# JANUS-Institute/HallThrusterPEM

Measured on AMD Instinct MI355X. Metric: coupled PEM-v0 model evals/sec, higher is better.
Workload: dtype f64

## Files before the change

### hallthrusterpem_amd/_lib.py

```python
import ctypes as C
import importlib.util
import os
import threading
from pathlib import Path

PKG = Path(__file__).resolve().parent
LIB_PATH = PKG / 'libpem_hip.so'

PEM_OK, PEM_ERR_INVALID_ARG, PEM_ERR_HIP, PEM_ERR_NO_DEVICE = 0, 1, 2, 3
NANGLE = 91
FUSED_LATENT_MAX_RANK = 8
FUSED_SYSTEM_MAX_RECORDS = 1024
FUSED_SYSTEM_MAX_RADII = 8
SYS_JION, SYS_VCC, SYS_T, SYS_UION = 0, 1, 2, 3
SWEEP_CATHODE, SWEEP_THRUSTER, SWEEP_PLUME = 0, 1, 2
DE_MAX_POP, DE_MAX_DIM = 1024, 16
DE_BEST1BIN, DE_RAND1BIN = 0, 1
CHAIN_TIME_BLOCK = 4096
MARGINALS_MAX_PAR, MARGINALS_MAX_BINS = 32, 64
HIST_ROW_TILE = 128
KDE_MAX_GRID, KDE_ROW_BLOCK = 4096, 4096

_dp = C.c_void_p
_sz = C.c_size_t
_f8 = C.c_double

SIGNATURES = {
    'pem_version': (C.c_char_p, []),
    'pem_last_error': (C.c_char_p, []),
    'pem_device_count': (C.c_int, []),
    'pem_init': (C.c_int, [C.c_int]),
    'pem_synchronize': (C.c_int, [_dp]),
    'pem_set_lanes_per_sample': (C.c_int, [C.c_int]),
    'pem_angle_grid': (C.POINTER(C.c_double), []),
    'pem_persistent_grid': (C.c_int, [_sz, C.c_int, C.c_int, C.c_int, C.POINTER(_sz), C.POINTER(_sz)]),
    'pem_coupled_occupancy': (C.c_int, [C.c_int, C.POINTER(C.c_int), C.POINTER(C.c_int)]),
    'pem_cathode_f64_dev': (C.c_int, [_sz] + [_dp] * 6 + [_f8, _dp, _dp]),
    'pem_cathode_f64': (C.c_int, [_sz] + [_dp] * 6 + [_f8, _dp]),
    'pem_plume_f64_dev': (C.c_int, [_sz, C.c_int, _dp, _f8] + [_dp] * 10 + [_dp] * 4 + [_dp]),
    'pem_plume_f64': (C.c_int, [_sz, C.c_int, _dp, _f8] + [_dp] * 10 + [_dp] * 4),
    'pem_thruster_f64_dev': (C.c_int, [_sz] + [_dp] * 4 + [_dp] * 8 + [_dp]),
    'pem_thruster_f64': (C.c_int, [_sz] + [_dp] * 4 + [_dp] * 8),
    'pem_thruster_uion_f64_dev': (C.c_int, [_sz, _dp, _f8, _f8, C.c_int, _dp, _dp, _dp]),
    'pem_thruster_filter_f64_dev': (C.c_int, [_sz, C.c_int, _dp, _dp, _f8, C.c_int, _dp, _dp, _dp, _dp]),
    'pem_coupled_f64_dev': (C.c_int, [_sz, _f8, _f8] + [_dp] * 15 + [_dp] * 7 + [_dp]),
    'pem_coupled_f64': (C.c_int, [_sz, _f8, _f8] + [_dp] * 15 + [_dp] * 7),
    'pem_coupled_tiled_f64_dev': (C.c_int, [_sz, _f8, _f8, _dp] + [_dp] * 7 + [_dp]),
    'pem_coupled_mixed_dev': (C.c_int, [_sz, _f8, _f8] + [_dp] * 15 + [_dp] * 7 + [_dp]),
    'pem_coupled_loglik_f64_dev': (C.c_int, [_sz, _f8, _f8] + [_dp] * 15 + [C.c_int, C.c_int] + [_dp] * 4 + [_dp] * 5 + [_dp]),
    'pem_coupled_system_loglik_f64_dev': (C.c_int, [_sz, _f8, _f8] + [_dp] * 15 + [C.c_int, C.c_int, _dp, _dp, C.c_int, _dp, _f8, _f8, C.c_int]
                                          + [_dp] * 5 + [_dp]),
    'pem_coupled_system_predict_f64_dev': (C.c_int, [_sz, _f8, _f8] + [_dp] * 15 + [C.c_int, C.c_int, _dp, _dp, C.c_int, _dp, _f8, _f8, C.c_int]
                                           + [_dp] * 4 + [_sz, _dp, _dp]),
    'pem_coupled_system_loglik_radii_f64_dev': (C.c_int, [_sz, _f8, C.c_int, _dp] + [_dp] * 15
                                                + [C.c_int, C.c_int, _dp, _dp, C.c_int, _dp, _f8, _f8, C.c_int] + [_dp] * 5 + [_dp]),
    'pem_coupled_system_predict_radii_f64_dev': (C.c_int, [_sz, _f8, C.c_int, _dp] + [_dp] * 15
                                                 + [C.c_int, C.c_int, _dp, _dp, C.c_int, _dp, _f8, _f8, C.c_int] + [_dp] * 4 + [_sz, _dp, _dp]),
    'pem_predictive_inputs_f64_dev': (C.c_int, [_sz, C.c_int, C.c_uint64, C.c_uint64, C.c_uint32, _dp, _dp, _dp, _dp, _dp, _sz, C.c_int,
                                                _dp, C.c_uint32, _dp, _sz, _dp]),
    'pem_predictive_noise_f64_dev': (C.c_int, [_sz, C.c_int, _dp, _sz, _dp, C.c_uint64, C.c_uint64, C.c_uint32, _dp, _sz, _dp]),
    'pem_coupled_latent_f64_dev': (C.c_int, [_sz, _f8, _f8] + [_dp] * 15 + [C.c_int, C.c_int, _dp, _dp] + [_dp] * 4 + [_dp]),
    'pem_loglik_marginal_f64_dev': (C.c_int, [_sz, C.c_int, C.c_int, _dp, _dp, _dp, _f8, _f8, _dp, _dp, _dp]),
    'pem_log_prior_f64_dev': (C.c_int, [_sz, C.c_int, _dp, _dp, _dp, _dp, _dp, _dp, _dp, _dp]),
    'pem_jion_loglik_f64_dev': (C.c_int, [_sz, C.c_int, C.c_int] + [_dp] * 6 + [_dp]),
    'pem_svd_compress_f64_dev': (C.c_int, [_sz, C.c_int, C.c_int, C.c_int, _f8, _dp, _dp, _dp, _dp]),
    'pem_svd_reconstruct_f64_dev': (C.c_int, [_sz, C.c_int, C.c_int, C.c_int, _f8, _dp, _dp, _dp, _dp]),
    'pem_coupled_mc_f64_dev': (C.c_int, [_sz, C.c_uint64, C.c_uint64, C.c_uint32, C.c_int, _dp, _dp, _dp, _f8, _f8, _dp, _sz] + [_dp] * 7 + [_dp]),
    'pem_sparse_predict_f64_dev': (C.c_int, [_sz, C.c_int, C.c_int, _dp, _dp, _dp, C.c_int, _dp, _sz, _dp, _sz, C.c_int, C.c_int, _dp]),
    'pem_sparse_grid_values_f64_dev': (C.c_int, [_sz, C.c_int, C.c_int, _dp, _dp, _dp, C.c_int, _dp, _sz, _dp, _sz, C.c_int, C.c_int, _dp]),
    'pem_sparse_predict_field_f64_dev': (C.c_int, [_sz, C.c_int, C.c_int, _dp, _dp, _dp, C.c_int, _dp, _sz, _dp, _sz, C.c_int, C.c_int,
                                                   C.c_int, C.c_int, C.c_int, C.c_int, C.c_double, _dp, _dp, _dp]),
    'pem_sparse_predict_chain_f64_dev': (C.c_int, [_sz, C.c_int, C.c_int, C.c_int, _dp, _f8, _f8, _f8, _f8, _dp, _sz, _dp, _sz,
                                                   C.c_int, C.c_int, C.c_int, C.c_int, C.c_double, _dp, _dp, _dp]),
    'pem_chain_system_loglik_f64_dev': (C.c_int, [_sz, C.c_int, C.c_int, C.c_int, _dp, _f8, _f8, _f8, _f8, _dp, _sz,
                                                  C.c_int, C.c_int, C.c_int, C.c_int, C.c_double, _dp, C.c_int, C.c_int, _dp, _dp,
                                                  _dp, _f8, _f8, _dp, _dp, _sz, _dp, _sz, _dp]),
    'pem_sparse_predict_chain_fields_f64_dev': (C.c_int, [_sz, C.c_int, C.c_int, C.c_int, _dp, _f8, _f8, _f8, _f8, _dp, _sz, _dp, _sz,
                                                          C.c_int, C.c_int, C.c_int, C.c_int, C.c_double, _dp, _dp,
                                                          C.c_int, C.c_int, C.c_int, C.c_int, C.c_double, _dp, _dp, _dp]),
    'pem_chain_fields_loglik_f64_dev': (C.c_int, [_sz, C.c_int, C.c_int, C.c_int, _dp, _f8, _f8, _f8, _f8, _dp, _sz,
                                                  C.c_int, C.c_int, C.c_int, C.c_int, C.c_double, _dp, C.c_int, C.c_int, _dp, _dp,
                                                  _dp, _f8, _f8, _dp, _dp, _sz, _dp, _sz,
                                                  C.c_int, C.c_int, C.c_int, C.c_int, C.c_double, _dp, C.c_int, _dp, _dp, _dp]),
    'pem_key_minmax_f64_dev': (C.c_int, [_sz, C.c_int, _dp, _sz, _dp, _dp, _dp, _dp]),
    'pem_range_hist_f64_dev': (C.c_int, [_sz, C.c_int, _dp, _sz, C.c_int, _dp, _dp, C.c_int, _dp, _dp]),
    'pem_range_narrow_dev': (C.c_int, [C.c_int, C.c_int, _dp, _dp, _dp, _dp, _dp]),
    'pem_qsel_bins': (C.c_int, [C.c_int, C.c_int, C.POINTER(C.c_int), C.POINTER(C.c_int)]),
    'pem_qsel_minmax_f64_dev': (C.c_int, [_sz, C.c_int, _dp, _sz, _dp, _dp, _dp, _dp]),
    'pem_qsel_hist1_f64_dev': (C.c_int, [_sz, C.c_int, _dp, _sz, _dp, _dp, C.c_int, _dp, _dp]),
# ... 71 lines not shown
        if _lib is not None:
            return _lib
        path = Path(os.environ.get('PEM_HIP_LIB', LIB_PATH))
        if 'PEM_HIP_LIB' not in os.environ:
            from . import build as _build
            if _build.needs_build():
                if _build.have_hipcc():
                    _build.build()
                elif not path.exists():
                    raise RuntimeError('libpem_hip.so is missing and hipcc is not available to build it')
                else:
                    import warnings
                    warnings.warn('libpem_hip.so is older than its sources and hipcc is not available: loading the stale library')
        _hip_runtime = _share_torch_hip_runtime()
        lib = C.CDLL(str(path))
        for name, (res, args) in SIGNATURES.items():
            fn = getattr(lib, name)
            fn.restype = res
            fn.argtypes = args
        _lib = lib
    return _lib


def check(rc: int):
    if rc != PEM_OK:
        raise PemHipError(rc, load().pem_last_error().decode(errors='replace'))


def device_count() -> int:
    return int(load().pem_device_count())


def set_device(index: int):
    check(load().pem_init(int(index)))
    try:
        import torch
        torch.cuda.set_device(int(index))
    except ImportError:
        pass


def persistent_grid(n: int, cus: int, wg_per_cu: int, memory_bound: bool = True):
    wg, spr = _sz(0), _sz(0)
    check(load().pem_persistent_grid(int(n), int(cus), int(wg_per_cu), 1 if memory_bound else 0, C.byref(wg), C.byref(spr)))
    return int(wg.value), int(spr.value)


def coupled_occupancy(profile_mode: int = 1):
    cus, per = C.c_int(0), C.c_int(0)
    check(load().pem_coupled_occupancy(int(profile_mode), C.byref(cus), C.byref(per)))
    return int(cus.value), int(per.value)


def require_device():
    if device_count() < 1:
        raise PemHipError(PEM_ERR_NO_DEVICE, 'no HIP device visible; hallthrusterpem_amd has no CPU path')
```

### hallthrusterpem_amd/csrc/pem_kernels.hip

```cpp
#include <cmath>
#include <cstdlib>
#include <atomic>
#include <mutex>
#include <type_traits>

#include "pem_math.h"
#include "pem_philox.h"
#include "pem_plume.h"

namespace {

using namespace pem;
using namespace pem_model;

struct CoupledIO {
    const double *V_a, *T_e, *V_vac, *Pstar, *P_T, *mdot_a, *a_1;
    double *V_cc, *I_B0, *T;
};

struct McDesign {
    unsigned long long seed, first;
    unsigned int stream;
    int swap_dim;
    int kind[15];
// ... 50 lines not shown
        v.x6 = cio.a_1[gi];
    } else {
        v.x0 = io.I_B0[gi];
        v.x1 = io.T ? io.T[gi] : 0.0;
        v.x2 = v.x3 = v.x4 = v.x5 = v.x6 = 0.0;
    }
    return v;
}

__device__ __attribute__((noinline)) double transform_call(int kind, double a, double b, double u) {
    return pem::transform(kind, a, b, u);
}

constexpr int MC_LDS_DOUBLES = 48;
__device__ __forceinline__ SampleIn<true> generate_sample(const McDesign& mc, const double* design, long long g_local) {
    const int* design_kind = reinterpret_cast<const int*>(design + 32);
    const unsigned long long g = mc.first + (unsigned long long)g_local;
    const unsigned int k0 = (unsigned int)mc.seed, k1 = (unsigned int)(mc.seed >> 32);
    double x[16];
    double u[16];
#pragma unroll
    for (int pair = 0; pair < 8; ++pair) {
        const unsigned int st0 = mc.stream + ((mc.swap_dim == -2 || mc.swap_dim == 2 * pair) ? 1u : 0u);
        const unsigned int st1 = mc.stream + ((mc.swap_dim == -2 || mc.swap_dim == 2 * pair + 1) ? 1u : 0u);
        const pem::Philox4 r = pem::philox4x32_10((unsigned int)g, (unsigned int)(g >> 32), (unsigned int)pair, st0, k0, k1);
        pem::Philox4 r1 = r;
        if (2 * pair + 1 < 15 && st1 != st0)
            r1 = pem::philox4x32_10((unsigned int)g, (unsigned int)(g >> 32), (unsigned int)pair, st1, k0, k1);
        u[2 * pair] = pem::u53(r.x, r.y);
        u[2 * pair + 1] = pem::u53(r1.z, r1.w);
    }
#pragma unroll
    for (int d = 0; d < 15; ++d) x[d] = transform_call(__builtin_amdgcn_readfirstlane(design_kind[d]), design[d], design[15 + d], u[d]);
    if (mc.x_out) {
#pragma unroll
        for (int d = 0; d < 15; ++d) mc.x_out[(size_t)d * mc.ld + g_local] = x[d];
    }
    SampleIn<true> v;
    v.P_b = x[0]; v.x0 = x[1]; v.x1 = x[2]; v.x2 = x[3]; v.x3 = x[4]; v.x4 = x[5]; v.x5 = x[6]; v.x6 = x[7];
    v.c0 = x[8]; v.c1 = x[9]; v.c2 = x[10]; v.c3 = x[11]; v.c4 = x[12]; v.c5 = x[13]; v.sigma = x[14];
    return v;
}

constexpr int NPARAM = 9;
constexpr int WPB = 4;
template <int L>
constexpr int param_rows() { return 2 * L > NPARAM ? 2 * L : NPARAM; }
constexpr int QPOLY_DOUBLES = (PEM_NDI + PEM_NQB) * PEM_NDC * 2;
template <int L, int JMODE>
constexpr int wave_lds_doubles() {
    return param_rows<L>() * WAVE +
           ((JMODE == 1 || JMODE == 3 || JMODE == 4 || JMODE == 5 || JMODE == 6 || JMODE == 7 || JMODE == 8 || JMODE == 9) ? (WAVE / L) * NANG + 2 : JMODE == 2 ? ((WAVE / L) * NANG + 4) / 2 : 0);
}
template <int L, int JMODE>
constexpr int fast_lds_doubles() { return TABLE_DOUBLES + WPB * wave_lds_doubles<L, JMODE>(); }

#ifndef PEM_LOGLIK_MU
#define PEM_LOGLIK_MU 2
#endif

struct WaveLds {
    const double* meas;
    const int2* span;
    const double* unode;
    int n_unode;
    double* pred;
    long long ld_pred;
    const double* rtab;
    double2* pairs;
    int n_radii;
    const double2* simpson;
    const double* poly;
    const double2* qpoly;
    double* params;
    double* tile;
    unsigned tile_off;
};

struct ChunkSums {
    double den, num, lo;
};
template <typename JT, bool WRITE_J>
__device__ __attribute__((noinline)) ChunkSums exact_chunk(double X1a, double X2a, double jcex, double a1, double a2, int k0,
                                                           int nk, const double2* w, JT* tile_row) {
#pragma clang fp contract(off)
    ChunkSums r{0.0, 0.0, __builtin_inf()};
    for (int j = 0; j < nk; ++j) {
        const int k = k0 + j;
        if (k >= NANG) break;
        const double alpha = k == NANG - 1 ? HALF_PI : (double)k * GRID_H;
        const double t1 = alpha / a1, t2 = alpha / a2;
        const double f = X1a * exp(-(t1 * t1)) + X2a * exp(-(t2 * t2));
        const double ji = f + jcex;
        if (WRITE_J) tile_row[j] = (JT)ji;
        r.lo = fmin(r.lo, WRITE_J ? ji : f);
        r.den = __builtin_fma(w[j].x, f, r.den);
        r.num = __builtin_fma(w[j].y, f, r.num);
    }
    return r;
}

struct CountCtx {
    pem::Record* rec;
    uint8_t* row_certain;
    uint8_t* row_uncertain;
    unsigned cap;
    unsigned tab_off;
    unsigned below_off;
// ... 512 lines not shown
        simpson_functionals(m.qpoly, fabs(a1), u1, d1, n1);
        simpson_functionals(m.qpoly, fabs(a2), u2, d2, n2);
        den = plain ? fma(base * A1, d1, (base * A2) * d2) : den;
        num = plain ? fma(base * A1, n1, (base * A2) * n2) : num;
    }

    double cos_div = num / den;
    if (cos_div == __builtin_inf()) cos_div = __builtin_nan("");
    if constexpr (JMODE == 4 || JMODE == 5) {
        if (live && (!__builtin_isfinite(den) || !__builtin_isfinite(j_cex))) atomicOr(io.q.flags + 1, 1);
    }
    if constexpr (JMODE == 3) {
        if (live) io.loglik[g] = params[(2 * L) * WAVE + lane];
    }
    if constexpr (JMODE == 6 || JMODE == 8) {
        if (live) {
            const unsigned cond = ((unsigned)((t * WAVE) % io.n_cond) + (unsigned)lane) % (unsigned)io.n_cond;
            io.loglik[g] = system_epilogue_sum(params[(2 * L) * WAVE + lane], m, cond, V_cc, thrust, v_exh);
        }
    }
    if constexpr (PREDICT) {
        if (live) {
            const unsigned u = (unsigned)((t * WAVE) % io.n_cond) + (unsigned)lane;
            system_epilogue_store(m, u % (unsigned)io.n_cond, V_cc, thrust, v_exh, pred_row(m, t, u, io.n_cond));
        }
    }
    if (live) {
        if (!PREDICT || io.div) io.div[g] = acos(cos_div);
        if (have_T && (!PREDICT || io.Tc)) io.Tc[g] = thrust * cos_div;
        if (io.invalid) io.invalid[g] = (uint8_t)((inv_mask >> lane) & 1);
        if constexpr (COUPLED) {
            if (!PREDICT || cio.V_cc) cio.V_cc[g] = V_cc;
            if (cio.I_B0) cio.I_B0[g] = I_B0;
            if (cio.T) cio.T[g] = thrust;
        }
    }
    wave_lds_sync();
}

template <int JMODE, bool MC>
constexpr int min_waves_per_simd() { return (MC && JMODE == 0) ? 3 : 1; }

struct NoDesign {};
template <bool MC, int JMODE = 0>
using DesignArg = typename std::conditional<
    MC, McDesign,
    typename std::conditional<JMODE == 6, SystemTable,
                              typename std::conditional<JMODE == 7, SystemPredict,
                                                        typename std::conditional<JMODE >= 8, SystemRadii, NoDesign>::type>::type>::type>::type;

template <int NQ, bool PM>
constexpr int count_lds_bytes() { return NANG * NQ * 8 + NQ * NANG * 4 + 8 + (PM ? NANG * 16 + 8 : 0) + WPB * (int)sizeof(CountCtx); }

template <int L, bool COUPLED, int JMODE, bool MC = false, int NQ = 0, bool PM = false>
__global__ __launch_bounds__(WAVE * WPB) __attribute__((amdgpu_waves_per_eu(min_waves_per_simd<JMODE, MC>())))
void plume_r1_kernel(PlumeIO io, CoupledIO cio, long long ntiles, DesignArg<MC, JMODE> mc) {
    static_assert(!MC || COUPLED, "the fused Monte-Carlo mode generates the coupled inputs");
    static_assert((JMODE == 4 || JMODE == 5) == (NQ > 0), "the counting modes, and only they, know their number of brackets");
    static_assert(NQ == 0 || L == 4, "count_round keeps one bit per sample of a 16-sample round");
    static_assert(L == 2 || L == 4 || L == 8, "lanes per sample");
    extern __shared__ __attribute__((aligned(16))) unsigned char smem_raw[];
    double* lds = reinterpret_cast<double*>(smem_raw);
    double2* tab_simpson = reinterpret_cast<double2*>(lds);
    double* tab_poly = lds + 2 * NSIMP;
    const int tid = threadIdx.x, wave = tid >> 6, lane = tid & 63;
    WaveLds m;
    m.simpson = tab_simpson;
    m.poly = tab_poly;
    m.params = lds + TABLE_DOUBLES + wave * wave_lds_doubles<L, JMODE>();
    m.tile = m.params + param_rows<L>() * WAVE;
    m.tile_off = (unsigned)(reinterpret_cast<unsigned char*>(m.tile) - smem_raw);
    m.qpoly = nullptr;
    if constexpr (JMODE == 0) {
        double* q = lds + TABLE_DOUBLES + WPB * wave_lds_doubles<L, JMODE>();
        for (int i = tid; i < QPOLY_DOUBLES; i += WAVE * WPB) q[i] = PEM_QPOLY[i];
        m.qpoly = reinterpret_cast<const double2*>(q);
    }
    double* design = nullptr;
    if constexpr (MC) {
        static_assert(!MC || JMODE == 0 || JMODE == 1 || JMODE == 4 || JMODE == 5, "the fused Monte-Carlo mode writes an fp64 profile or none");
        design = lds + TABLE_DOUBLES + WPB * wave_lds_doubles<L, JMODE>() + (JMODE == 0 ? QPOLY_DOUBLES : 0);
        if (tid < 15) {
            design[tid] = mc.a[tid];
            design[15 + tid] = mc.b[tid];
            reinterpret_cast<int*>(design + 32)[tid] = mc.kind[tid];
        }
    }
    m.meas = nullptr;
    if constexpr (JMODE == 3) {
        double* meas = lds + TABLE_DOUBLES + WPB * wave_lds_doubles<L, JMODE>();
        const int nent = io.n_cond * io.n_ang;
        for (int i = tid; i < nent; i += WAVE * WPB) {
            const int r = 4 * ((i / io.n_ang) * (io.n_ang | 1) + i % io.n_ang);
            meas[r] = io.m_wgt[i];
            meas[r + 1] = io.m_y[i];
            meas[r + 2] = io.m_inv_std[i];
            meas[r + 3] = __longlong_as_double((long long)io.m_kidx[i]);
        }
        m.meas = meas;
    }
    m.span = nullptr;
    m.unode = nullptr;
    m.n_unode = 0;
    m.pred = nullptr;
    m.ld_pred = 0;
    m.rtab = nullptr;
    m.pairs = nullptr;
    m.n_radii = 0;
    if constexpr (JMODE == 6 || JMODE == 7 || JMODE == 8 || JMODE == 9) {
        double* meas = lds + TABLE_DOUBLES + WPB * wave_lds_doubles<L, JMODE>();
        for (int i = tid; i < 4 * mc.n_rec; i += WAVE * WPB) meas[i] = mc.rec[i];
        int2* span = reinterpret_cast<int2*>(meas + 4 * mc.n_rec);
        for (int i = tid; i < 4 * io.n_cond; i += WAVE * WPB) {
            const int first = min(max(mc.span[2 * i], 0), mc.n_rec);
            span[i] = make_int2(first, min(max(mc.span[2 * i + 1], 0), mc.n_rec - first));
        }
        double* unode = reinterpret_cast<double*>(span + 4 * io.n_cond);
        for (int i = tid; i < (mc.n_node > 2 ? mc.n_node : 2); i += WAVE * WPB)
            unode[i] = i < mc.n_node ? uion_den(uion_z(mc.z0, mc.z1, mc.ncells, min(max(mc.node[i], 0), mc.ncells - 1)))
                                     : __builtin_nan("");
        m.meas = meas;
        m.span = span;
        m.unode = unode;
        m.n_unode = mc.n_node;
        if constexpr (JMODE == 7 || JMODE == 9) {
            m.pred = mc.pred;
            m.ld_pred = mc.ld_pred;
        }
        if constexpr (JMODE == 8 || JMODE == 9) {
            const int nr = min(max(mc.n_radii, 1), SYS_RADII_MAX);
            double* rtab = unode + (((mc.n_node > 2 ? mc.n_node : 2) + 1) & ~1);
            if (tid < nr) {
                const double r = mc.radii[tid];
                rtab[3 * tid] = r;
                rtab[3 * tid + 1] = 1.0 / (r * r);
                rtab[3 * tid + 2] = 1.0 / (2.0 * PEM_PI * (r * r));
            }
            m.rtab = rtab;
            m.pairs = reinterpret_cast<double2*>(rtab + ((3 * nr + 1) & ~1)) + wave * (WAVE / L) * nr;
            m.n_radii = nr;
        }
    }

    using QC = typename std::conditional<(NQ > 0), QCount, NoCount>::type;
    QC qc;
    if constexpr (NQ > 0) {
        double* qbase = lds + TABLE_DOUBLES + WPB * wave_lds_doubles<L, JMODE>() + (MC ? MC_LDS_DOUBLES : 0);
        uint2* qtab = reinterpret_cast<uint2*>(qbase);
        unsigned* qbelow = reinterpret_cast<unsigned*>(qtab + NANG * NQ);
        for (int i = tid; i < NANG * NQ; i += WAVE * WPB) {
            const int c = i / NQ, q = i - c * NQ;
            qtab[i] = q < io.q.nq ? make_uint2(io.q.br[c * io.q.nq + q].loh, io.q.br[c * io.q.nq + q].words) : make_uint2(0xffffffffu, 0u);
            qbelow[i] = 0;
        }
        const unsigned gw = blockIdx.x * WPB + wave;
        unsigned char* after = reinterpret_cast<unsigned char*>(qbelow + NQ * NANG);
        after = reinterpret_cast<unsigned char*>((reinterpret_cast<uintptr_t>(after) + 15) & ~uintptr_t(15));
        unsigned pm_off = 0;
        if constexpr (PM) {
            uint4* pmt = reinterpret_cast<uint4*>(after);
            for (int i = tid; i < NANG; i += WAVE * WPB) pmt[i] = io.q.premask[i];
            pm_off = (unsigned)(after - smem_raw);
            after += NANG * sizeof(uint4);
        }
        CountCtx* ctx = reinterpret_cast<CountCtx*>(after) + wave;
        if (lane == 0) {
            ctx->rec = io.q.rec + (size_t)gw * io.q.cap;
            ctx->row_certain = io.q.row_certain;
            ctx->row_uncertain = io.q.row_uncertain;
            ctx->cap = io.q.cap;
            ctx->tab_off = (unsigned)(reinterpret_cast<unsigned char*>(qtab) - smem_raw);
            ctx->below_off = (unsigned)(reinterpret_cast<unsigned char*>(qbelow) - smem_raw);
            ctx->pm_off = pm_off;
        }
        qc.ctx_off = (unsigned)(reinterpret_cast<unsigned char*>(ctx) - smem_raw);
        qc.below_off = (unsigned)(reinterpret_cast<unsigned char*>(qbelow) - smem_raw);
        qc.cap = io.q.cap;
        qc.cnt = 0;
    }
    for (int i = tid; i < NSIMP; i += WAVE * WPB)
        tab_simpson[i] = i < NANG ? make_double2(PEM_SIMPSON_CDEN[i], PEM_SIMPSON_CNUM[i]) : make_double2(0.0, 0.0);
    for (int i = tid; i < PEM_NDI * PEM_NDC; i += WAVE * WPB) tab_poly[i] = PEM_DPOLY[i];
    __syncthreads();

    const double rad = io.radius;
    const double inv_r2 = 1.0 / (rad * rad);
    const double inv_2pi_r2 = 1.0 / (2.0 * PEM_PI * (rad * rad));

    const long long nfull = io.n / WAVE;
    const bool one_tile_per_wave = (long long)gridDim.x * WPB >= ntiles;
    const long long vblock = ((JMODE == 1 || JMODE == 2) && one_tile_per_wave) ? (long long)pem::xcd_contiguous_block() : (long long)blockIdx.x;
    const long long me = vblock * WPB + wave, nwaves = (long long)gridDim.x * WPB;
    long long t = me;
    if constexpr (MC) {
        for (; t < nfull; t += nwaves) {
            const SampleIn<COUPLED> in = generate_sample(mc, design, t * WAVE + lane);
            process_tile<L, COUPLED, JMODE, true, NQ, PM>(io, cio, m, in, t, lane, rad, inv_r2, inv_2pi_r2, qc);
        }
        if (nfull < ntiles && (nfull % nwaves) == me) {
            const long long g = nfull * WAVE + lane;
            McDesign quiet = mc;
            if (g >= io.n) quiet.x_out = nullptr;
            const SampleIn<COUPLED> in = generate_sample(quiet, design, g < io.n ? g : io.n - 1);
            process_tile<L, COUPLED, JMODE, false, NQ, PM>(io, cio, m, in, nfull, lane, rad, inv_r2, inv_2pi_r2, qc);
        }
    } else {
        if (t < nfull) {
            SampleIn<COUPLED> nxt = load_sample<COUPLED>(io, cio, t * WAVE + lane);
            for (; t < nfull; t += nwaves) {
                const SampleIn<COUPLED> in = nxt;
                if (t + nwaves < nfull) nxt = load_sample<COUPLED>(io, cio, (t + nwaves) * WAVE + lane);
                process_tile<L, COUPLED, JMODE, true, NQ, PM>(io, cio, m, in, t, lane, rad, inv_r2, inv_2pi_r2, qc);
            }
        }
        if (nfull < ntiles && (nfull % nwaves) == me) {
            const long long g = nfull * WAVE + lane;
            const SampleIn<COUPLED> in = load_sample<COUPLED>(io, cio, g < io.n ? g : io.n - 1);
            process_tile<L, COUPLED, JMODE, false, NQ, PM>(io, cio, m, in, nfull, lane, rad, inv_r2, inv_2pi_r2, qc);
        }
    }
    if constexpr (NQ > 0) {
        if (lane == 0) {
            io.q.rec_count[blockIdx.x * WPB + wave] = qc.cnt;
            if (qc.cnt > qc.cap) atomicOr(io.q.flags, 1);
        }
        __syncthreads();
        for (int i = tid; i < NQ * NANG; i += WAVE * WPB) {
            const int q = i / NANG, c = i - q * NANG;
            const unsigned v = reinterpret_cast<const unsigned*>(smem_raw + qc.below_off)[i];
            if (v && q < io.q.nq) atomicAdd(&io.q.below[c * io.q.nq + q], (unsigned long long)v);
        }
    }
}

std::atomic<int> g_lanes{4};
double g_angle_grid[NANG];
std::once_flag g_grid_once;

constexpr long long ONE_SHOT_ROUNDS = 3;
long long persistent_grid(long long ntiles, long long cus, long long per_cu, bool memory_bound) {
    if (per_cu < 1) per_cu = 1;
    long long g = cus * per_cu;
    const long long need = (ntiles + WPB - 1) / WPB;
    if (g > need) g = need;
    if (!memory_bound) return g;
    if (need > ONE_SHOT_ROUNDS * g) return need;
    return (long long)balanced_grid((size_t)need, (size_t)g);
}

int fast_grid(long long per_cu, long long ntiles, bool memory_bound, unsigned* grid) {
    int cus = 0;
    HIP_TRY(pem::device_cus(&cus));
    if (const char* e = getenv("PEM_WAVES_PER_CU")) {
        const long long v = atoll(e) / WPB;
        if (v >= 1 && v < per_cu) per_cu = v;
    }
    *grid = (unsigned)persistent_grid(ntiles, cus, per_cu, memory_bound);
    if (const char* e = getenv("PEM_GRID_MULT")) {
        const long long m = atoll(e), need = (ntiles + WPB - 1) / WPB, cap = (long long)cus * (per_cu < 1 ? 1 : per_cu);
        *grid = (unsigned)((m <= 0 || m * cap > need) ? need : m * cap);
    }
    return PEM_OK;
}

size_t system_lds_bytes(int n_cond, const SystemTable& tab) {
    return (size_t)tab.n_rec * 32 + (size_t)n_cond * 32 + (size_t)(tab.n_node > 2 ? tab.n_node : 2) * 8;
}

size_t radii_lds_bytes(int n_cond, const SystemRadii& tab, int samples_per_round) {
    return ((system_lds_bytes(n_cond, tab) + 15) & ~(size_t)15) + (size_t)((3 * tab.n_radii + 1) & ~1) * 8 +
           (size_t)WPB * samples_per_round * tab.n_radii * 16;
}

template <int L, int JMODE, bool MC, int NQ = 0, bool PM = false>
size_t r1_lds_bytes(const PlumeIO& io) {
    size_t lds = (size_t)fast_lds_doubles<L, JMODE>() * 8;
    if (NQ > 0) lds += (size_t)count_lds_bytes<(NQ > 0 ? NQ : 1), PM>();
    if (JMODE == 3) lds += (size_t)io.n_cond * (io.n_ang | 1) * 32;
    if (JMODE == 0) lds += (size_t)QPOLY_DOUBLES * 8;
    if (MC) lds += (size_t)MC_LDS_DOUBLES * 8;
    return lds;
}

template <int L, bool COUPLED, int JMODE, bool MC, int NQ = 0, bool PM = false>
int r1_per_cu(size_t lds, long long* per_cu) {
    auto kern = plume_r1_kernel<L, COUPLED, JMODE, MC, NQ, PM>;
    static std::once_flag once;
    static int by_regs = 0;
    static hipError_t err = hipSuccess;
    std::call_once(once, [&] {
        hipFuncAttributes fa;
        err = hipFuncGetAttributes(&fa, reinterpret_cast<const void*>(kern));
        if (err != hipSuccess) return;
        const int regs = fa.numRegs > 0 ? ((fa.numRegs + 7) & ~7) : 256;
        by_regs = (512 / regs) * 4 / WPB;
    });
    HIP_TRY(err);
    long long v = (long long)(160 * 1024 / lds);
    const int cap = (JMODE == 0 ? 12 : 8) / WPB;
    if (v > by_regs) v = by_regs;
    if (v > cap) v = cap;
    *per_cu = v;
    return PEM_OK;
}

template <int L, bool COUPLED, int JMODE, bool MC = false, int NQ = 0, bool PM = false>
int launch_r1(const PlumeIO& io, const CoupledIO& cio, hipStream_t st, const McDesign& mc = McDesign{}, unsigned* grid_only = nullptr,
              const SystemTable* sys = nullptr, const SystemPredict* pr = nullptr, const SystemRadii* rd = nullptr) {
    size_t lds = r1_lds_bytes<L, JMODE, MC, NQ, PM>(io);
    if constexpr (JMODE == 6) lds += system_lds_bytes(io.n_cond, *sys);
    if constexpr (JMODE == 7) lds += system_lds_bytes(io.n_cond, *pr);
    if constexpr (JMODE == 8 || JMODE == 9) lds += radii_lds_bytes(io.n_cond, *rd, WAVE / L);
    const long long ntiles = (io.n + WAVE - 1) / WAVE;
    unsigned grid = 0;
    auto kern = plume_r1_kernel<L, COUPLED, JMODE, MC, NQ, PM>;
    if (lds > 64 * 1024) {
        static pem::LdsAttrOnce attr;
        HIP_TRY(attr.ensure(reinterpret_cast<const void*>(kern)));
    }
    long long per_cu = 0;
    if (int rc = r1_per_cu<L, COUPLED, JMODE, MC, NQ, PM>(lds, &per_cu)) return rc;
    if (int rc = fast_grid(per_cu, ntiles, JMODE == 1 || JMODE == 2, &grid)) return rc;
    if (grid_only) {
        *grid_only = grid;
        return PEM_OK;
    }
    if constexpr (MC) hipLaunchKernelGGL(kern, dim3(grid), dim3(WAVE * WPB), lds, st, io, cio, ntiles, mc);
    else if constexpr (JMODE == 6) hipLaunchKernelGGL(kern, dim3(grid), dim3(WAVE * WPB), lds, st, io, cio, ntiles, *sys);
    else if constexpr (JMODE == 7) hipLaunchKernelGGL(kern, dim3(grid), dim3(WAVE * WPB), lds, st, io, cio, ntiles, *pr);
    else if constexpr (JMODE == 8 || JMODE == 9) hipLaunchKernelGGL(kern, dim3(grid), dim3(WAVE * WPB), lds, st, io, cio, ntiles, *rd);
    else hipLaunchKernelGGL(kern, dim3(grid), dim3(WAVE * WPB), lds, st, io, cio, ntiles, NoDesign{});
    HIP_TRY(hipGetLastError());
    return PEM_OK;
}

template <bool COUPLED, int JMODE>
int dispatch_lanes(const PlumeIO& io, const CoupledIO& cio, hipStream_t st) {
    switch (g_lanes.load(std::memory_order_relaxed)) {
        case 2: return launch_r1<2, COUPLED, JMODE>(io, cio, st);
        case 8: return launch_r1<8, COUPLED, JMODE>(io, cio, st);
        default: return launch_r1<4, COUPLED, JMODE>(io, cio, st);
    }
}

}

namespace pem {
char* error_buffer() {
    thread_local char buf[512] = "";
    return buf;
}
}

extern "C" {

const char* pem_last_error(void) { return pem::error_buffer(); }

int pem_set_lanes_per_sample(int lanes) {
    if (lanes == 0) lanes = 4;
    if (lanes == 2 || lanes == 4 || lanes == 8) g_lanes = lanes;
    return g_lanes;
}

int pem_persistent_grid(size_t n, int cus, int wg_per_cu, int memory_bound, size_t* workgroups, size_t* samples_per_round) {
    if (!workgroups || !samples_per_round) return fail(PEM_ERR_INVALID_ARG, "pem_persistent_grid: NULL result pointer");
    if (cus < 1 || wg_per_cu < 1) return fail(PEM_ERR_INVALID_ARG, "pem_persistent_grid: cus and wg_per_cu must be positive");
    const long long ntiles = (long long)((n + WAVE - 1) / WAVE);
    const long long g = persistent_grid(ntiles, cus, wg_per_cu, memory_bound != 0);
    const long long resident = g < (long long)cus * wg_per_cu ? g : (long long)cus * wg_per_cu;
    *workgroups = (size_t)g;
    *samples_per_round = (size_t)resident * WPB * WAVE;
    return PEM_OK;
}

int pem_coupled_occupancy(int profile_mode, int* cus, int* wg_per_cu) {
    if (!cus || !wg_per_cu) return fail(PEM_ERR_INVALID_ARG, "pem_coupled_occupancy: NULL result pointer");
    if (int rc = check_device()) return rc;
    HIP_TRY(pem::device_cus(cus));
    PlumeIO io{};
    long long v = 0;
    int rc;
#define PEM_OCC(L_)                                                                                      \
    (profile_mode == 0   ? r1_per_cu<L_, true, 0, false>(r1_lds_bytes<L_, 0, false>(io), &v)               \
     : profile_mode == 1 ? r1_per_cu<L_, true, 1, false>(r1_lds_bytes<L_, 1, false>(io), &v)               \
                         : r1_per_cu<L_, true, 2, false>(r1_lds_bytes<L_, 2, false>(io), &v))
    if (profile_mode < 0 || profile_mode > 2) return fail(PEM_ERR_INVALID_ARG, "pem_coupled_occupancy: profile_mode must be 0, 1 or 2");
    switch (g_lanes.load(std::memory_order_relaxed)) {
        case 2: rc = PEM_OCC(2); break;
        case 8: rc = PEM_OCC(8); break;
        default: rc = PEM_OCC(4); break;
    }
#undef PEM_OCC
    if (rc) return rc;
    if (const char* e = getenv("PEM_WAVES_PER_CU")) {
        const long long w = atoll(e) / WPB;
        if (w >= 1 && w < v) v = w;
    }
    *wg_per_cu = (int)v;
    return PEM_OK;
}

const double* pem_angle_grid(void) {
    std::call_once(g_grid_once, [] {
        const double step = HALF_PI / 90.0;
        for (int k = 0; k < NANG; ++k) g_angle_grid[k] = (double)k * step;
        g_angle_grid[NANG - 1] = HALF_PI;
    });
    return g_angle_grid;
}

int pem_plume_f64_dev(size_t n, int n_radii, const double* radii, double torr2pa, const double* P_b, const double* c0,
                      const double* c1, const double* c2, const double* c3, const double* c4, const double* c5,
                      const double* sigma_cex, const double* I_B0, const double* T, double* j_ion, double* div_angle,
                      double* T_c, uint8_t* invalid, pem_stream_t stream) {
    if (n_radii < 1 || !radii) return fail(PEM_ERR_INVALID_ARG, "pem_plume: need at least one sweep radius");
    if (n == 0) return PEM_OK;
    if (!P_b || !c0 || !c1 || !c2 || !c3 || !c4 || !c5 || !sigma_cex || !I_B0 || !j_ion || !div_angle)
        return fail(PEM_ERR_INVALID_ARG, "pem_plume: NULL array");
    if ((T == nullptr) != (T_c == nullptr)) return fail(PEM_ERR_INVALID_ARG, "pem_plume: T and T_c go together");
    if (int rc = check_device()) return rc;
    hipStream_t st = static_cast<hipStream_t>(stream);
    PlumeIO io{(long long)n, torr2pa, radii[0], P_b, c0, c1, c2, c3, c4, c5, sigma_cex, I_B0, T, j_ion, div_angle, T_c, invalid};
    if (n_radii == 1 && aligned16(j_ion)) return dispatch_lanes<false, 1>(io, CoupledIO{}, st);
    return pem::launch_plume_radii(n, n_radii, radii, io, st);
}

int pem_coupled_f64_dev(size_t n, double torr2pa, double radius, const double* P_b, const double* V_a, const double* T_e,
                        const double* V_vac, const double* Pstar, const double* P_T, const double* mdot_a,
                        const double* a_1, const double* c0, const double* c1, const double* c2, const double* c3,
                        const double* c4, const double* c5, const double* sigma_cex, double* V_cc, double* I_B0,
                        double* T, double* j_ion, double* div_angle, double* T_c, uint8_t* invalid, pem_stream_t stream) {
    if (n == 0) return PEM_OK;
    if (!P_b || !V_a || !T_e || !V_vac || !Pstar || !P_T || !mdot_a || !a_1 || !c0 || !c1 || !c2 || !c3 || !c4 || !c5 ||
        !sigma_cex || !V_cc || !div_angle || !T_c)
        return fail(PEM_ERR_INVALID_ARG, "pem_coupled: NULL array");
    if (j_ion && !aligned16(j_ion)) return fail(PEM_ERR_INVALID_ARG, "pem_coupled: j_ion must be 16-byte aligned");
    if (int rc = check_device()) return rc;
    hipStream_t st = static_cast<hipStream_t>(stream);
    PlumeIO io{(long long)n, torr2pa, radius, P_b, c0, c1, c2, c3, c4, c5, sigma_cex, nullptr, nullptr, j_ion, div_angle, T_c, invalid};
    CoupledIO cio{V_a, T_e, V_vac, Pstar, P_T, mdot_a, a_1, V_cc, I_B0, T};
    return j_ion ? dispatch_lanes<true, 1>(io, cio, st) : dispatch_lanes<true, 0>(io, cio, st);
}

int pem_coupled_tiled_f64_dev(size_t n, double torr2pa, double radius, const double* x_tiled, double* V_cc, double* I_B0,
                              double* T, double* j_ion, double* div_angle, double* T_c, uint8_t* invalid, pem_stream_t stream) {
    if (n == 0) return PEM_OK;
    if (!x_tiled || !V_cc || !div_angle || !T_c) return fail(PEM_ERR_INVALID_ARG, "pem_coupled_tiled: NULL array");
    if (j_ion && !aligned16(j_ion)) return fail(PEM_ERR_INVALID_ARG, "pem_coupled_tiled: j_ion must be 16-byte aligned");
    if (int rc = check_device()) return rc;
    hipStream_t st = static_cast<hipStream_t>(stream);
    const double* x = x_tiled;
// ... 276 lines not shown
```

### include/pem_hip.h

```cpp
#ifndef PEM_HIP_H
#define PEM_HIP_H

#include <stddef.h>
#include <stdint.h>

#ifdef __cplusplus
extern "C" {
#endif

#define PEM_NANGLE 91

#define PEM_OK 0
#define PEM_ERR_INVALID_ARG 1
#define PEM_ERR_HIP 2
#define PEM_ERR_NO_DEVICE 3

typedef void* pem_stream_t;

const char* pem_version(void);
const char* pem_last_error(void);
int pem_device_count(void);
int pem_init(int device);
int pem_synchronize(pem_stream_t stream);
int pem_set_lanes_per_sample(int lanes);
const double* pem_angle_grid(void);
int pem_persistent_grid(size_t n, int cus, int wg_per_cu, int memory_bound, size_t* workgroups, size_t* samples_per_round);
int pem_coupled_occupancy(int profile_mode, int* cus, int* wg_per_cu);

int pem_cathode_f64_dev(size_t n, const double* P_b, const double* V_a, const double* T_e,
                        const double* V_vac, const double* Pstar, const double* P_T, double torr2pa,
                        double* V_cc, pem_stream_t stream);
int pem_cathode_f64(size_t n, const double* P_b, const double* V_a, const double* T_e,
                    const double* V_vac, const double* Pstar, const double* P_T, double torr2pa,
                    double* V_cc);

int pem_plume_f64_dev(size_t n, int n_radii, const double* radii, double torr2pa, const double* P_b,
                      const double* c0, const double* c1, const double* c2, const double* c3,
                      const double* c4, const double* c5, const double* sigma_cex, const double* I_B0,
                      const double* T, double* j_ion, double* div_angle, double* T_c, uint8_t* invalid,
                      pem_stream_t stream);
int pem_plume_f64(size_t n, int n_radii, const double* radii, double torr2pa, const double* P_b,
                  const double* c0, const double* c1, const double* c2, const double* c3,
                  const double* c4, const double* c5, const double* sigma_cex, const double* I_B0,
                  const double* T, double* j_ion, double* div_angle, double* T_c, uint8_t* invalid);

int pem_thruster_f64_dev(size_t n, const double* V_a, const double* V_cc, const double* mdot_a,
                         const double* a_1, double* I_B0, double* I_d, double* T, double* eta_c,
                         double* eta_m, double* eta_v, double* eta_a, double* v_exh, pem_stream_t stream);
int pem_thruster_f64(size_t n, const double* V_a, const double* V_cc, const double* mdot_a,
                     const double* a_1, double* I_B0, double* I_d, double* T, double* eta_c,
                     double* eta_m, double* eta_v, double* eta_a, double* v_exh);

int pem_thruster_uion_f64_dev(size_t n, const double* v_exh, double z0, double z1, int ncells, double* z,
                              double* u_ion, pem_stream_t stream);
int pem_thruster_filter_f64_dev(size_t n, int ncells, const double* u_ion, const double* z, double shock_threshold,
                                int use_shock, const double* T, const double* I_B0, uint8_t* flags,
                                pem_stream_t stream);

int pem_coupled_f64_dev(size_t n, double torr2pa, double radius, const double* P_b, const double* V_a,
                        const double* T_e, const double* V_vac, const double* Pstar, const double* P_T,
                        const double* mdot_a, const double* a_1, const double* c0, const double* c1,
                        const double* c2, const double* c3, const double* c4, const double* c5,
                        const double* sigma_cex, double* V_cc, double* I_B0, double* T, double* j_ion,
                        double* div_angle, double* T_c, uint8_t* invalid, pem_stream_t stream);
int pem_coupled_f64(size_t n, double torr2pa, double radius, const double* P_b, const double* V_a,
                    const double* T_e, const double* V_vac, const double* Pstar, const double* P_T,
                    const double* mdot_a, const double* a_1, const double* c0, const double* c1,
                    const double* c2, const double* c3, const double* c4, const double* c5,
                    const double* sigma_cex, double* V_cc, double* I_B0, double* T, double* j_ion,
                    double* div_angle, double* T_c, uint8_t* invalid);

int pem_coupled_tiled_f64_dev(size_t n, double torr2pa, double radius, const double* x_tiled, double* V_cc, double* I_B0,
                              double* T, double* j_ion, double* div_angle, double* T_c, uint8_t* invalid,
                              pem_stream_t stream);

int pem_coupled_mixed_dev(size_t n, double torr2pa, double radius, const double* P_b, const double* V_a,
                          const double* T_e, const double* V_vac, const double* Pstar, const double* P_T,
                          const double* mdot_a, const double* a_1, const double* c0, const double* c1,
                          const double* c2, const double* c3, const double* c4, const double* c5,
                          const double* sigma_cex, double* V_cc, double* I_B0, double* T, float* j_ion_f32,
// ... 256 lines not shown
```

Measured before the change: 6.455 billion.

## Hoist first sample load above table setup barrier and add narrow one-shot kernels

The plume kernel body becomes a template over workgroup width. The LDS table fill is staged through registers so the first sample's global load can be issued before the barrier, overlapping the load latency with table setup. Optional one- and two-wave one-shot kernel variants are added, with the one-wave variant laying the D-polynomial over its round tile to save LDS. A query for their occupancy is also added. The narrow variants are only used when selected by an environment variable or macro, and the hoisted load adds register pressure.

```diff
diff --git a/hallthrusterpem_amd/_lib.py b/hallthrusterpem_amd/_lib.py
--- a/hallthrusterpem_amd/_lib.py
+++ b/hallthrusterpem_amd/_lib.py
@@ -35,6 +35,7 @@
     'pem_angle_grid': (C.POINTER(C.c_double), []),
     'pem_persistent_grid': (C.c_int, [_sz, C.c_int, C.c_int, C.c_int, C.POINTER(_sz), C.POINTER(_sz)]),
     'pem_coupled_occupancy': (C.c_int, [C.c_int, C.POINTER(C.c_int), C.POINTER(C.c_int)]),
+    'pem_coupled_one_shot_occupancy': (C.c_int, [C.c_int, C.POINTER(C.c_int), C.POINTER(_sz)]),
     'pem_cathode_f64_dev': (C.c_int, [_sz] + [_dp] * 6 + [_f8, _dp, _dp]),
     'pem_cathode_f64': (C.c_int, [_sz] + [_dp] * 6 + [_f8, _dp]),
     'pem_plume_f64_dev': (C.c_int, [_sz, C.c_int, _dp, _f8] + [_dp] * 10 + [_dp] * 4 + [_dp]),
@@ -212,6 +213,12 @@
     return int(cus.value), int(per.value)
 
 
+def coupled_one_shot_occupancy(waves_per_wg: int = 0):
+    per, lds = C.c_int(0), _sz(0)
+    check(load().pem_coupled_one_shot_occupancy(int(waves_per_wg), C.byref(per), C.byref(lds)))
+    return int(per.value), int(lds.value)
+
+
 def require_device():
     if device_count() < 1:
         raise PemHipError(PEM_ERR_NO_DEVICE, 'no HIP device visible; hallthrusterpem_amd has no CPU path')
diff --git a/hallthrusterpem_amd/csrc/pem_kernels.hip b/hallthrusterpem_amd/csrc/pem_kernels.hip
--- a/hallthrusterpem_amd/csrc/pem_kernels.hip
+++ b/hallthrusterpem_amd/csrc/pem_kernels.hip
@@ -126,8 +126,15 @@
     return param_rows<L>() * WAVE +
            ((JMODE == 1 || JMODE == 3 || JMODE == 4 || JMODE == 5 || JMODE == 6 || JMODE == 7 || JMODE == 8 || JMODE == 9) ? (WAVE / L) * NANG + 2 : JMODE == 2 ? ((WAVE / L) * NANG + 4) / 2 : 0);
 }
-template <int L, int JMODE>
-constexpr int fast_lds_doubles() { return TABLE_DOUBLES + WPB * wave_lds_doubles<L, JMODE>(); }
+template <int L, int JMODE, int W = WPB, bool SHARE = false>
+constexpr int fast_lds_doubles() { return TABLE_DOUBLES - (SHARE ? PEM_NDI * PEM_NDC : 0) + W * wave_lds_doubles<L, JMODE>(); }
+
+#ifndef PEM_HOIST_LOAD
+#define PEM_HOIST_LOAD 1
+#endif
+#ifndef PEM_W1_SHARE
+#define PEM_W1_SHARE 1
+#endif
 
 #ifndef PEM_LOGLIK_MU
 #define PEM_LOGLIK_MU 2
@@ -746,9 +753,11 @@
 template <int NQ, bool PM>
 constexpr int count_lds_bytes() { return NANG * NQ * 8 + NQ * NANG * 4 + 8 + (PM ? NANG * 16 + 8 : 0) + WPB * (int)sizeof(CountCtx); }
 
-template <int L, bool COUPLED, int JMODE, bool MC = false, int NQ = 0, bool PM = false>
-__global__ __launch_bounds__(WAVE * WPB) __attribute__((amdgpu_waves_per_eu(min_waves_per_simd<JMODE, MC>())))
-void plume_r1_kernel(PlumeIO io, CoupledIO cio, long long ntiles, DesignArg<MC, JMODE> mc) {
+template <int W, bool SHARE, int L, bool COUPLED, int JMODE, bool MC, int NQ, bool PM>
+__device__ __forceinline__ void plume_r1_body(const PlumeIO& io, const CoupledIO& cio, long long ntiles, const DesignArg<MC, JMODE>& mc) {
+    static_assert(W == WPB || (JMODE == 1 && !MC && NQ == 0), "the tables behind the per-wave regions are laid out for WPB waves");
+    static_assert(!SHARE || W == 1, "only a workgroup of one wave may lay the D-polynomial over its round tile");
+    static_assert(!SHARE || (WAVE / L) * NANG + 2 >= PEM_NDI * PEM_NDC, "the round tile holds the D-polynomial");
     static_assert(!MC || COUPLED, "the fused Monte-Carlo mode generates the coupled inputs");
     static_assert((JMODE == 4 || JMODE == 5) == (NQ > 0), "the counting modes, and only they, know their number of brackets");
     static_assert(NQ == 0 || L == 4, "count_round keeps one bit per sample of a 16-sample round");
@@ -756,24 +765,24 @@
     extern __shared__ __attribute__((aligned(16))) unsigned char smem_raw[];
     double* lds = reinterpret_cast<double*>(smem_raw);
     double2* tab_simpson = reinterpret_cast<double2*>(lds);
-    double* tab_poly = lds + 2 * NSIMP;
     const int tid = threadIdx.x, wave = tid >> 6, lane = tid & 63;
     WaveLds m;
     m.simpson = tab_simpson;
+    m.params = lds + (SHARE ? 2 * NSIMP : TABLE_DOUBLES) + wave * wave_lds_doubles<L, JMODE>();
+    m.tile = m.params + param_rows<L>() * WAVE;
+    double* tab_poly = SHARE ? m.tile : lds + 2 * NSIMP;
     m.poly = tab_poly;
-    m.params = lds + TABLE_DOUBLES + wave * wave_lds_doubles<L, JMODE>();
-    m.tile = m.params + param_rows<L>() * WAVE;
     m.tile_off = (unsigned)(reinterpret_cast<unsigned char*>(m.tile) - smem_raw);
     m.qpoly = nullptr;
     if constexpr (JMODE == 0) {
-        double* q = lds + TABLE_DOUBLES + WPB * wave_lds_doubles<L, JMODE>();
-        for (int i = tid; i < QPOLY_DOUBLES; i += WAVE * WPB) q[i] = PEM_QPOLY[i];
+        double* q = lds + TABLE_DOUBLES + W * wave_lds_doubles<L, JMODE>();
+        for (int i = tid; i < QPOLY_DOUBLES; i += WAVE * W) q[i] = PEM_QPOLY[i];
         m.qpoly = reinterpret_cast<const double2*>(q);
     }
     double* design = nullptr;
     if constexpr (MC) {
         static_assert(!MC || JMODE == 0 || JMODE == 1 || JMODE == 4 || JMODE == 5, "the fused Monte-Carlo mode writes an fp64 profile or none");
-        design = lds + TABLE_DOUBLES + WPB * wave_lds_doubles<L, JMODE>() + (JMODE == 0 ? QPOLY_DOUBLES : 0);
+        design = lds + TABLE_DOUBLES + W * wave_lds_doubles<L, JMODE>() + (JMODE == 0 ? QPOLY_DOUBLES : 0);
         if (tid < 15) {
             design[tid] = mc.a[tid];
             design[15 + tid] = mc.b[tid];
@@ -782,9 +791,9 @@
     }
     m.meas = nullptr;
     if constexpr (JMODE == 3) {
-        double* meas = lds + TABLE_DOUBLES + WPB * wave_lds_doubles<L, JMODE>();
+        double* meas = lds + TABLE_DOUBLES + W * wave_lds_doubles<L, JMODE>();
         const int nent = io.n_cond * io.n_ang;
-        for (int i = tid; i < nent; i += WAVE * WPB) {
+        for (int i = tid; i < nent; i += WAVE * W) {
             const int r = 4 * ((i / io.n_ang) * (io.n_ang | 1) + i % io.n_ang);
             meas[r] = io.m_wgt[i];
             meas[r + 1] = io.m_y[i];
@@ -802,15 +811,15 @@
     m.pairs = nullptr;
     m.n_radii = 0;
     if constexpr (JMODE == 6 || JMODE == 7 || JMODE == 8 || JMODE == 9) {
-        double* meas = lds + TABLE_DOUBLES + WPB * wave_lds_doubles<L, JMODE>();
-        for (int i = tid; i < 4 * mc.n_rec; i += WAVE * WPB) meas[i] = mc.rec[i];
+        double* meas = lds + TABLE_DOUBLES + W * wave_lds_doubles<L, JMODE>();
+        for (int i = tid; i < 4 * mc.n_rec; i += WAVE * W) meas[i] = mc.rec[i];
         int2* span = reinterpret_cast<int2*>(meas + 4 * mc.n_rec);
-        for (int i = tid; i < 4 * io.n_cond; i += WAVE * WPB) {
+        for (int i = tid; i < 4 * io.n_cond; i += WAVE * W) {
             const int first = min(max(mc.span[2 * i], 0), mc.n_rec);
             span[i] = make_int2(first, min(max(mc.span[2 * i + 1], 0), mc.n_rec - first));
         }
         double* unode = reinterpret_cast<double*>(span + 4 * io.n_cond);
-        for (int i = tid; i < (mc.n_node > 2 ? mc.n_node : 2); i += WAVE * WPB)
+        for (int i = tid; i < (mc.n_node > 2 ? mc.n_node : 2); i += WAVE * W)
             unode[i] = i < mc.n_node ? uion_den(uion_z(mc.z0, mc.z1, mc.ncells, min(max(mc.node[i], 0), mc.ncells - 1)))
                                      : __builtin_nan("");
         m.meas = meas;
@@ -839,21 +848,21 @@
     using QC = typename std::conditional<(NQ > 0), QCount, NoCount>::type;
     QC qc;
     if constexpr (NQ > 0) {
-        double* qbase = lds + TABLE_DOUBLES + WPB * wave_lds_doubles<L, JMODE>() + (MC ? MC_LDS_DOUBLES : 0);
+        double* qbase = lds + TABLE_DOUBLES + W * wave_lds_doubles<L, JMODE>() + (MC ? MC_LDS_DOUBLES : 0);
         uint2* qtab = reinterpret_cast<uint2*>(qbase);
         unsigned* qbelow = reinterpret_cast<unsigned*>(qtab + NANG * NQ);
-        for (int i = tid; i < NANG * NQ; i += WAVE * WPB) {
+        for (int i = tid; i < NANG * NQ; i += WAVE * W) {
             const int c = i / NQ, q = i - c * NQ;
             qtab[i] = q < io.q.nq ? make_uint2(io.q.br[c * io.q.nq + q].loh, io.q.br[c * io.q.nq + q].words) : make_uint2(0xffffffffu, 0u);
             qbelow[i] = 0;
         }
-        const unsigned gw = blockIdx.x * WPB + wave;
+        const unsigned gw = blockIdx.x * W + wave;
         unsigned char* after = reinterpret_cast<unsigned char*>(qbelow + NQ * NANG);
         after = reinterpret_cast<unsigned char*>((reinterpret_cast<uintptr_t>(after) + 15) & ~uintptr_t(15));
         unsigned pm_off = 0;
         if constexpr (PM) {
             uint4* pmt = reinterpret_cast<uint4*>(after);
-            for (int i = tid; i < NANG; i += WAVE * WPB) pmt[i] = io.q.premask[i];
+            for (int i = tid; i < NANG; i += WAVE * W) pmt[i] = io.q.premask[i];
             pm_off = (unsigned)(after - smem_raw);
             after += NANG * sizeof(uint4);
         }
@@ -872,20 +881,46 @@
         qc.cap = io.q.cap;
         qc.cnt = 0;
     }
-    for (int i = tid; i < NSIMP; i += WAVE * WPB)
-        tab_simpson[i] = i < NANG ? make_double2(PEM_SIMPSON_CDEN[i], PEM_SIMPSON_CNUM[i]) : make_double2(0.0, 0.0);
-    for (int i = tid; i < PEM_NDI * PEM_NDC; i += WAVE * WPB) tab_poly[i] = PEM_DPOLY[i];
+    const long long nfull = io.n / WAVE;
+    const bool one_tile_per_wave = (long long)gridDim.x * W >= ntiles;
+    const long long vblock = ((JMODE == 1 || JMODE == 2) && one_tile_per_wave) ? (long long)pem::xcd_contiguous_block() : (long long)blockIdx.x;
+    const long long me = vblock * W + wave, nwaves = (long long)gridDim.x * W;
+    long long t = me;
+    constexpr bool HOIST = !MC && PEM_HOIST_LOAD;
+    constexpr int NT = WAVE * W, SIMP_IT = (NSIMP + NT - 1) / NT, POLY_IT = (PEM_NDI * PEM_NDC + NT - 1) / NT;
+    double2 stage_s[SIMP_IT];
+    double stage_p[POLY_IT];
+#pragma unroll
+    for (int k = 0; k < SIMP_IT; ++k) {
+        const int i = tid + k * NT;
+        const int j = i < NANG ? i : NANG - 1;
+        stage_s[k] = make_double2(i < NANG ? PEM_SIMPSON_CDEN[j] : 0.0, i < NANG ? PEM_SIMPSON_CNUM[j] : 0.0);
+    }
+#pragma unroll
+    for (int k = 0; k < POLY_IT; ++k) {
+        const int i = tid + k * NT;
+        stage_p[k] = PEM_DPOLY[i < PEM_NDI * PEM_NDC ? i : PEM_NDI * PEM_NDC - 1];
+    }
+    SampleIn<COUPLED> first_in;
+    if constexpr (HOIST) {
+        if (t < nfull) first_in = load_sample<COUPLED>(io, cio, t * WAVE + lane);
+    }
+#pragma unroll
+    for (int k = 0; k < SIMP_IT; ++k) {
+        const int i = tid + k * NT;
+        if (i < NSIMP) tab_simpson[i] = stage_s[k];
+    }
+#pragma unroll
+    for (int k = 0; k < POLY_IT; ++k) {
+        const int i = tid + k * NT;
+        if (i < PEM_NDI * PEM_NDC) tab_poly[i] = stage_p[k];
+    }
     __syncthreads();
 
     const double rad = io.radius;
     const double inv_r2 = 1.0 / (rad * rad);
     const double inv_2pi_r2 = 1.0 / (2.0 * PEM_PI * (rad * rad));
 
-    const long long nfull = io.n / WAVE;
-    const bool one_tile_per_wave = (long long)gridDim.x * WPB >= ntiles;
-    const long long vblock = ((JMODE == 1 || JMODE == 2) && one_tile_per_wave) ? (long long)pem::xcd_contiguous_block() : (long long)blockIdx.x;
-    const long long me = vblock * WPB + wave, nwaves = (long long)gridDim.x * WPB;
-    long long t = me;
     if constexpr (MC) {
         for (; t < nfull; t += nwaves) {
             const SampleIn<COUPLED> in = generate_sample(mc, design, t * WAVE + lane);
@@ -900,7 +935,8 @@
         }
     } else {
         if (t < nfull) {
-            SampleIn<COUPLED> nxt = load_sample<COUPLED>(io, cio, t * WAVE + lane);
+            SampleIn<COUPLED> nxt;
+            if constexpr (HOIST) nxt = first_in; else nxt = load_sample<COUPLED>(io, cio, t * WAVE + lane);
             for (; t < nfull; t += nwaves) {
                 const SampleIn<COUPLED> in = nxt;
                 if (t + nwaves < nfull) nxt = load_sample<COUPLED>(io, cio, (t + nwaves) * WAVE + lane);
@@ -915,16 +951,31 @@
     }
     if constexpr (NQ > 0) {
         if (lane == 0) {
-            io.q.rec_count[blockIdx.x * WPB + wave] = qc.cnt;
+            io.q.rec_count[blockIdx.x * W + wave] = qc.cnt;
             if (qc.cnt > qc.cap) atomicOr(io.q.flags, 1);
         }
         __syncthreads();
-        for (int i = tid; i < NQ * NANG; i += WAVE * WPB) {
+        for (int i = tid; i < NQ * NANG; i += WAVE * W) {
             const int q = i / NANG, c = i - q * NANG;
             const unsigned v = reinterpret_cast<const unsigned*>(smem_raw + qc.below_off)[i];
             if (v && q < io.q.nq) atomicAdd(&io.q.below[c * io.q.nq + q], (unsigned long long)v);
         }
     }
+}
+
+template <int L, bool COUPLED, int JMODE, bool MC = false, int NQ = 0, bool PM = false>
+__global__ __launch_bounds__(WAVE * WPB) __attribute__((amdgpu_waves_per_eu(min_waves_per_simd<JMODE, MC>())))
+void plume_r1_kernel(PlumeIO io, CoupledIO cio, long long ntiles, DesignArg<MC, JMODE> mc) {
+    plume_r1_body<WPB, false, L, COUPLED, JMODE, MC, NQ, PM>(io, cio, ntiles, mc);
+}
+
+template <int W, int L, bool COUPLED>
+constexpr int narrow_waves_per_simd() { return (W == 2 && L == 2 && COUPLED) ? 1 : 2; }
+template <int W, int L, bool COUPLED, int JMODE>
+__global__ __launch_bounds__(WAVE * W) __attribute__((amdgpu_waves_per_eu(narrow_waves_per_simd<W, L, COUPLED>())))
+void plume_r1_kernel_narrow(PlumeIO io, CoupledIO cio, long long ntiles, NoDesign mc) {
+    static_assert(W == 1 || W == 2, "narrow workgroups");
+    plume_r1_body<W, W == 1 && PEM_W1_SHARE, L, COUPLED, JMODE, false, 0, false>(io, cio, ntiles, mc);
 }
 
 std::atomic<int> g_lanes{4};
@@ -942,7 +993,7 @@
     return (long long)balanced_grid((size_t)need, (size_t)g);
 }
 
-int fast_grid(long long per_cu, long long ntiles, bool memory_bound, unsigned* grid) {
+int fast_grid(long long per_cu, long long ntiles, bool memory_bound, unsigned* grid, bool* one_shot = nullptr) {
     int cus = 0;
     HIP_TRY(pem::device_cus(&cus));
     if (const char* e = getenv("PEM_WAVES_PER_CU")) {
@@ -950,11 +1001,26 @@
         if (v >= 1 && v < per_cu) per_cu = v;
     }
     *grid = (unsigned)persistent_grid(ntiles, cus, per_cu, memory_bound);
+    const long long need = (ntiles + WPB - 1) / WPB, cap = (long long)cus * (per_cu < 1 ? 1 : per_cu);
+    bool forced = false;
     if (const char* e = getenv("PEM_GRID_MULT")) {
-        const long long m = atoll(e), need = (ntiles + WPB - 1) / WPB, cap = (long long)cus * (per_cu < 1 ? 1 : per_cu);
+        const long long m = atoll(e);
         *grid = (unsigned)((m <= 0 || m * cap > need) ? need : m * cap);
-    }
+        forced = m <= 0;
+    }
+    if (one_shot) *one_shot = (long long)*grid == need && (need > cap || forced);
     return PEM_OK;
+}
+
+#ifndef PEM_ONE_SHOT_WAVES
+#define PEM_ONE_SHOT_WAVES 4
+#endif
+int one_shot_waves() {
+    if (const char* e = getenv("PEM_WAVES_PER_WG")) {
+        const int w = atoi(e);
+        if (w == 1 || w == 2 || w == WPB) return w;
+    }
+    return PEM_ONE_SHOT_WAVES;
 }
 
 size_t system_lds_bytes(int n_cond, const SystemTable& tab) {
@@ -998,6 +1064,16 @@
     return PEM_OK;
 }
 
+template <int W, int L, bool COUPLED>
+int launch_r1_narrow(const PlumeIO& io, const CoupledIO& cio, long long ntiles, hipStream_t st) {
+    constexpr size_t lds = (size_t)fast_lds_doubles<L, 1, W, W == 1 && PEM_W1_SHARE>() * 8;
+    static_assert(lds <= 64 * 1024, "no attribute needed for this much dynamic LDS");
+    const unsigned grid = (unsigned)((ntiles + W - 1) / W);
+    hipLaunchKernelGGL((plume_r1_kernel_narrow<W, L, COUPLED, 1>), dim3(grid), dim3(WAVE * W), lds, st, io, cio, ntiles, NoDesign{});
+    HIP_TRY(hipGetLastError());
+    return PEM_OK;
+}
+
 template <int L, bool COUPLED, int JMODE, bool MC = false, int NQ = 0, bool PM = false>
 int launch_r1(const PlumeIO& io, const CoupledIO& cio, hipStream_t st, const McDesign& mc = McDesign{}, unsigned* grid_only = nullptr,
               const SystemTable* sys = nullptr, const SystemPredict* pr = nullptr, const SystemRadii* rd = nullptr) {
@@ -1014,7 +1090,15 @@
     }
     long long per_cu = 0;
     if (int rc = r1_per_cu<L, COUPLED, JMODE, MC, NQ, PM>(lds, &per_cu)) return rc;
-    if (int rc = fast_grid(per_cu, ntiles, JMODE == 1 || JMODE == 2, &grid)) return rc;
+    bool one_shot = false;
+    if (int rc = fast_grid(per_cu, ntiles, JMODE == 1 || JMODE == 2, &grid, &one_shot)) return rc;
+    if constexpr (JMODE == 1 && !MC && NQ == 0) {
+        if (one_shot && !grid_only) {
+            const int w = one_shot_waves();
+            if (w == 1) return launch_r1_narrow<1, L, COUPLED>(io, cio, ntiles, st);
+            if (w == 2) return launch_r1_narrow<2, L, COUPLED>(io, cio, ntiles, st);
+        }
+    }
     if (grid_only) {
         *grid_only = grid;
         return PEM_OK;
@@ -1091,6 +1175,36 @@
         if (w >= 1 && w < v) v = w;
     }
     *wg_per_cu = (int)v;
+    return PEM_OK;
+}
+
+int pem_coupled_one_shot_occupancy(int waves_per_wg, int* wg_per_cu, size_t* lds_bytes) {
+    if (!wg_per_cu || !lds_bytes) return fail(PEM_ERR_INVALID_ARG, "pem_coupled_one_shot_occupancy: NULL result pointer");
+    if (waves_per_wg == 0) waves_per_wg = one_shot_waves();
+    if (waves_per_wg != 1 && waves_per_wg != 2 && waves_per_wg != WPB)
+        return fail(PEM_ERR_INVALID_ARG, "pem_coupled_one_shot_occupancy: waves_per_wg must be 0 (the width in effect), 1, 2 or %d", WPB);
+    if (int rc = check_device()) return rc;
+    int blocks = 0;
+#define PEM_OCC1(L_)                                                                                                              \
+    do {                                                                                                                          \
+        if (waves_per_wg == 1) {                                                                                                  \
+            *lds_bytes = (size_t)fast_lds_doubles<L_, 1, 1, PEM_W1_SHARE != 0>() * 8;                                             \
+            HIP_TRY(hipOccupancyMaxActiveBlocksPerMultiprocessor(&blocks, plume_r1_kernel_narrow<1, L_, true, 1>, WAVE, *lds_bytes)); \
+        } else if (waves_per_wg == 2) {                                                                                           \
+            *lds_bytes = (size_t)fast_lds_doubles<L_, 1, 2, false>() * 8;                                                         \
+            HIP_TRY(hipOccupancyMaxActiveBlocksPerMultiprocessor(&blocks, plume_r1_kernel_narrow<2, L_, true, 1>, 2 * WAVE, *lds_bytes)); \
+        } else {                                                                                                                  \
+            *lds_bytes = (size_t)fast_lds_doubles<L_, 1>() * 8;                                                                   \
+            HIP_TRY(hipOccupancyMaxActiveBlocksPerMultiprocessor(&blocks, plume_r1_kernel<L_, true, 1>, WPB * WAVE, *lds_bytes)); \
+        }                                                                                                                         \
+    } while (0)
+    switch (g_lanes.load(std::memory_order_relaxed)) {
+        case 2: PEM_OCC1(2); break;
+        case 8: PEM_OCC1(8); break;
+        default: PEM_OCC1(4); break;
+    }
+#undef PEM_OCC1
+    *wg_per_cu = blocks;
     return PEM_OK;
 }
 
diff --git a/include/pem_hip.h b/include/pem_hip.h
--- a/include/pem_hip.h
+++ b/include/pem_hip.h
@@ -26,6 +26,7 @@
 const double* pem_angle_grid(void);
 int pem_persistent_grid(size_t n, int cus, int wg_per_cu, int memory_bound, size_t* workgroups, size_t* samples_per_round);
 int pem_coupled_occupancy(int profile_mode, int* cus, int* wg_per_cu);
+int pem_coupled_one_shot_occupancy(int waves_per_wg, int* wg_per_cu, size_t* lds_bytes);
 
 int pem_cathode_f64_dev(size_t n, const double* P_b, const double* V_a, const double* T_e,
                         const double* V_vac, const double* Pstar, const double* P_T, double torr2pa,
```

New measurement: 6.488 billion (median of 6 runs). About the same (+0.5%).
